# XiaoshuiHuang/GMF

Measured on AMD Instinct MI355X. Metric: correspondences/sec (whole node), higher is better.
Workload: dtype f32 (split-fp16 MFMA operands, fp32 accumulate; the cross products of the attention's two contractions, S = K Q'^T and O = P V, on block-scaled e4m3 operands wherever the device-side score guard allows)

## Files before the change

### gmf_amd/csrc/encoder_h2.hip

```cpp
#include <algorithm>
#include <cstdlib>
#include "enc_common.hpp"
#include "enc_ff.hpp"
#include "launchers.hpp"

namespace gmf {

#ifndef GMF_H2_RING
#define GMF_H2_RING 2
#endif
constexpr int kRing = GMF_H2_RING;

template <int MODE>
GMF_DEVINL void front_h2_body(float* lds, const int bx, const int pair, const int zsel_in, const float* __restrict__ in,
                              const float* __restrict__ wst, const float* __restrict__ vecs, float* __restrict__ f_out,
                              float* __restrict__ q_out, float* __restrict__ k_out, float* __restrict__ v_out, int N, int tiles,
                              const PairTab* __restrict__ ptab = nullptr, unsigned* __restrict__ v_scale = nullptr,
                              const PvGuard guard = {}) {
  const int lane = threadIdx.x & 63, h = lane >> 5, i = lane & 31;
  const int wave = __builtin_amdgcn_readfirstlane(threadIdx.x >> 6);
  const size_t row0 = pair_row0(ptab, pair, N);
  N = pair_rows(ptab, pair, N);
  const int tiles_p = ptab ? (N + 31) >> 5 : tiles;
  if (bx * kWavesPerWG >= tiles_p) return;
// ... 845 lines not shown
#pragma unroll
      for (int r = 0; r < 16; ++r) y[mb][r] = (x1[16 * mb + r] + b[r]) * 256.0f;
    }
  }
  __syncthreads();
  ff_chunks<NP>(nx, y, lds, ff_wst, lvec_f + 2 * C, lvec_f + 2 * C + FFH, wave, lane, h, 0, FFH / 32);
#pragma unroll
  for (int mb = 0; mb < 4; ++mb) {
    float t[16];
#pragma unroll
    for (int r = 0; r < 16; ++r) t[r] = y[mb][r] * kH2Inv;
    if (active) store_block_p32(x2_out + toff, mb, t, lane);
  }
}

template <int NP, bool QSKIP = false, bool KVF = false>
__global__ void __launch_bounds__(256, 2)
k_linear_h2(const float* __restrict__ f_in, const float* __restrict__ front_wst, const float* __restrict__ front_vec,
            const float* __restrict__ ctx_img, const float* __restrict__ attn_wst, const float* __restrict__ attn_vec,
            const float* __restrict__ ff_wst, const float* __restrict__ ff_vec, float* __restrict__ q_out,
            float* __restrict__ k_out, float* __restrict__ v_out, float* __restrict__ x2_out, int N, int tiles, int T,
            int ttiles, const PairTab* __restrict__ ptab, unsigned* __restrict__ v_scale, const PvGuard guard,
            const float* __restrict__ kvf_wst, const float* __restrict__ kvf_bias) {
  __shared__ __attribute__((aligned(16))) float lds[kLinLdsFloats];
  tail_priority(blockIdx.y * gridDim.x + blockIdx.x, gridDim.x * gridDim.y);
  linear_h2_body<0, NP, QSKIP, KVF>(lds, f_in, front_wst, front_vec, ctx_img, attn_wst, attn_vec, ff_wst, ff_vec, q_out, k_out, v_out, x2_out, N,
                                    tiles, T, ttiles, ptab, v_scale, guard, kvf_wst, kvf_bias);
}

template <bool KVF>
__global__ void __launch_bounds__(256, 2)
k_linear_roles(const float* __restrict__ f_in, const float* __restrict__ front_wst, const float* __restrict__ front_vec,
               const float* __restrict__ ctx_img, const float* __restrict__ attn_wst, const float* __restrict__ attn_vec,
               const float* __restrict__ ff_wst, const float* __restrict__ ff_vec, float* __restrict__ q_out,
               float* __restrict__ k_out, float* __restrict__ v_out, float* __restrict__ x2_out, int N, int tiles, int T,
               int ttiles, unsigned* __restrict__ v_scale, const PvGuard guard, const PairTab* __restrict__ ptab,
               const float* __restrict__ kvf_wst, const float* __restrict__ kvf_bias) {
  __shared__ __attribute__((aligned(16))) float lds[kLinLdsFloats];
  if (blockIdx.z == 0)
    linear_h2_body<1, 3, false, KVF>(lds, f_in, front_wst, front_vec, ctx_img, attn_wst, attn_vec, ff_wst, ff_vec, q_out, k_out, v_out, x2_out, N,
                                     tiles, T, ttiles, ptab, v_scale, guard, kvf_wst, kvf_bias);
  else
    linear_h2_body<2>(lds, f_in, front_wst, front_vec, ctx_img, attn_wst, attn_vec, ff_wst, ff_vec, q_out, k_out, v_out, x2_out, N,
                      tiles, T, ttiles, ptab);
}

__global__ void __launch_bounds__(256)
k_ff_reduce(const float* __restrict__ part, const float* __restrict__ x1, const float* __restrict__ vecs,
            float* __restrict__ x2_out, int tiles, int hs) {
  const int lane = threadIdx.x & 63, h = lane >> 5;
  const int tile = blockIdx.x * kWavesPerWG + (threadIdx.x >> 6);
  if (tile >= tiles) return;
  const int mb = blockIdx.z;
// ... 24 lines not shown
hipError_t launch_front_h2(int mode, bool split, const float* in, const float* wst, const float* vecs, float* f, float* q, float* k,
                           float* v, int B, int N, int tiles, hipStream_t s, const PairTab* ptab, unsigned* v_scale, PvGuard guard) {
  dim3 g = tgrid(tiles, B);
  if (split) g.z = 3;
  if (mode == 3) { g.z = 1; hipLaunchKernelGGL(k_front_h2<3>, g, dim3(256), 0, s, in, wst, vecs, f, q, k, v, N, tiles, ptab, v_scale, guard); }
  else if (mode == 1) hipLaunchKernelGGL(k_front_h2<1>, g, dim3(256), 0, s, in, wst, vecs, f, q, k, v, N, tiles, ptab, v_scale, guard);
  else if (mode == 2) hipLaunchKernelGGL(k_front_h2<2>, g, dim3(256), 0, s, in, wst, vecs, f, q, k, v, N, tiles, ptab, v_scale, guard);
  else hipLaunchKernelGGL(k_front_h2<0>, g, dim3(256), 0, s, in, wst, vecs, f, q, k, v, N, tiles, ptab, v_scale, guard);
  return hipGetLastError();
}

hipError_t launch_linear_h2(bool roles, const float* f, const float* front_wst, const float* front_vec, const float* ctx_img,
                            const float* attn_wst, const float* attn_vec, const float* ff_wst, const float* ff_vec, float* q,
                            float* k, float* v, float* x2, int B, int N, int tiles, int T, int ttiles, hipStream_t s,
                            bool one_product, const PairTab* ptab, unsigned* v_scale, PvGuard guard, const float* kvf_wst,
                            const float* kvf_bias) {
  const float* const none = nullptr;
  if (roles && kvf_wst)
    hipLaunchKernelGGL(k_linear_roles<true>, tgrid(tiles, B, 2), dim3(256), 0, s, f, front_wst, front_vec, ctx_img, attn_wst, attn_vec,
                       ff_wst, ff_vec, q, k, v, x2, N, tiles, T, ttiles, v_scale, guard, ptab, kvf_wst, kvf_bias);
  else if (roles)
    hipLaunchKernelGGL(k_linear_roles<false>, tgrid(tiles, B, 2), dim3(256), 0, s, f, front_wst, front_vec, ctx_img, attn_wst, attn_vec,
                       ff_wst, ff_vec, q, k, v, x2, N, tiles, T, ttiles, v_scale, guard, ptab, none, none);
  else if (kvf_wst && !q)
    hipLaunchKernelGGL((k_linear_h2<3, true, true>), tgrid(tiles, B), dim3(256), 0, s, f, front_wst, front_vec, ctx_img, attn_wst, attn_vec, ff_wst,
                       ff_vec, q, k, v, x2, N, tiles, T, ttiles, ptab, v_scale, guard, kvf_wst, kvf_bias);
  else if (kvf_wst)
    hipLaunchKernelGGL((k_linear_h2<3, false, true>), tgrid(tiles, B), dim3(256), 0, s, f, front_wst, front_vec, ctx_img, attn_wst, attn_vec, ff_wst,
                       ff_vec, q, k, v, x2, N, tiles, T, ttiles, ptab, v_scale, guard, kvf_wst, kvf_bias);
  else if (one_product)
    hipLaunchKernelGGL(k_linear_h2<1>, tgrid(tiles, B), dim3(256), 0, s, f, front_wst, front_vec, ctx_img, attn_wst, attn_vec, ff_wst,
                       ff_vec, q, k, v, x2, N, tiles, T, ttiles, ptab, v_scale, guard, none, none);
  else if (!q)
    hipLaunchKernelGGL((k_linear_h2<3, true>), tgrid(tiles, B), dim3(256), 0, s, f, front_wst, front_vec, ctx_img, attn_wst, attn_vec, ff_wst,
                       ff_vec, q, k, v, x2, N, tiles, T, ttiles, ptab, v_scale, guard, none, none);
  else
    hipLaunchKernelGGL(k_linear_h2<3>, tgrid(tiles, B), dim3(256), 0, s, f, front_wst, front_vec, ctx_img, attn_wst, attn_vec, ff_wst,
                       ff_vec, q, k, v, x2, N, tiles, T, ttiles, ptab, v_scale, guard, none, none);
  return hipGetLastError();
}

hipError_t launch_ctx_prep_h2(bool pe, const float* ctx, const float* wst, const float* vecs, float* out, int B, int T,
                              int ttiles, int sets, int wst_stride, int vec_stride, hipStream_t s, bool rowmajor) {
  if (pe) hipLaunchKernelGGL(k_ctx_prep_h2<true>, tgrid(ttiles, B, sets), dim3(256), 0, s, ctx, wst, vecs, out, T, ttiles, wst_stride, vec_stride);
  else if (rowmajor) hipLaunchKernelGGL((k_ctx_prep_h2<false, true>), tgrid(ttiles, B, sets), dim3(256), 0, s, ctx, wst, vecs, out, T, ttiles, wst_stride, vec_stride);
  else hipLaunchKernelGGL(k_ctx_prep_h2<false>, tgrid(ttiles, B, sets), dim3(256), 0, s, ctx, wst, vecs, out, T, ttiles, wst_stride, vec_stride);
  return hipGetLastError();
}

hipError_t launch_fusion_attn_h2(bool pe, const float* x, const float* ctx_img, const float* wst, const float* vecs,
                                 float* x1, int B, int N, int tiles, int T, int ttiles, hipStream_t s, bool rowmajor) {
  if (pe) hipLaunchKernelGGL(k_fusion_attn_h2<true>, tgrid(tiles, B), dim3(256), 0, s, x, ctx_img, wst, vecs, x1, N, tiles, T, ttiles);
  else if (rowmajor) hipLaunchKernelGGL((k_fusion_attn_h2<false, true>), tgrid(tiles, B), dim3(256), 0, s, x, ctx_img, wst, vecs, x1, N, tiles, T, ttiles);
// ... 72 lines not shown
```

### gmf_amd/csrc/encoder_kernels.hip

```cpp
#include <algorithm>
#include <type_traits>
#include "enc_common.hpp"
#include "enc_ff.hpp"

namespace gmf {

template <int MODE>
__global__ void __launch_bounds__(256, 2)
k_front(const float* __restrict__ in, const float* __restrict__ wst, const float* __restrict__ vecs,
        float* __restrict__ f_out, float* __restrict__ q_out, float* __restrict__ k_out,
        float* __restrict__ v_out, int N, int tiles) {
  __shared__ __attribute__((aligned(16))) float lds[2 * kStageFloats];
  const int lane = threadIdx.x & 63, wave = threadIdx.x >> 6, h = lane >> 5, i = lane & 31;
  const int pair = blockIdx.y;
  const int tile_raw = blockIdx.x * kWavesPerWG + wave;
  const bool active = tile_raw < tiles;
  const int tile = active ? tile_raw : tiles - 1;
  const size_t toff = ((size_t)pair * tiles + tile) * (32 * C);

  constexpr bool FIRST = (MODE == 1);
  StageStream ss;
  if (MODE == 2) ss.init(lds, lds + kStageFloats, wave, kWavesPerWG, lane, wst + 4 * kStageFloats, 12);
  else ss.init(lds, lds + kStageFloats, wave, kWavesPerWG, lane, wst, 16);
  ss.prime();
// ... 1064 lines not shown
  ss.prime();
  const FusTile ft{fus + toff};
  if (next_wst) scattn_epilogue_h2<true>(o, active, ss, lvec, ft, out + toff, lane, h, lvec + 2 * C, stat_next, pair,
                                         tile_raw * 32 + (lane & 31) < N);
  else scattn_epilogue_h2<false>(o, active, ss, lvec, ft, out + toff, lane, h);
}

GMF_DEVINL bool attn_pv_on(const unsigned* __restrict__ v_scale, const PvGuard& guard, int bid, int n_items, int n_full, int ksplits,
                           int wgs_per_pair, const PairTab* __restrict__ ptab = nullptr) {
  if (!guard.stat) return v_scale != nullptr;
  const AttnItem it = attn_item(bid, n_items, n_full, ksplits);
  const int slot = it.valid ? it.item / wgs_per_pair : 0;
  return pv_planes_on(v_scale, guard, ptab ? ptab[slot].ord : slot);
}

template <int NPROD, int CFMT, bool PVF8 = false, bool FOLD = false>
__global__ void __launch_bounds__(256, 2)
k_scattn_h2p(const float* __restrict__ q_img, const float* __restrict__ k_img, const float* __restrict__ v_img,
             const float* __restrict__ fus, const float* __restrict__ wst, const float* __restrict__ vecs,
             float* out, int N, int tiles, int wgs_per_pair, const float* __restrict__ c_dense,
             int n_items, int n_full, int ksplits, float* __restrict__ part_o, float* __restrict__ part_ml,
             const float* __restrict__ next_wst, const float* __restrict__ next_bias, const PairTab* __restrict__ ptab,
             const unsigned* __restrict__ v_scale, const float* qf_img, const float* __restrict__ qw_wst,
             const float* __restrict__ qw_bias, const PvGuard guard, const float* __restrict__ kvf_vec) {
  __shared__ __attribute__((aligned(16))) float lds[4 * kStageFloats];
  tail_priority(blockIdx.x, gridDim.x);
  if (!PVF8 || attn_pv_on(v_scale, guard, blockIdx.x, n_items, n_full, ksplits, wgs_per_pair, ptab))
    scattn_h2p_body<NPROD, CFMT, 4, PVF8, FOLD>(lds, blockIdx.x, q_img, k_img, v_img, fus, wst, vecs, out, N, tiles, wgs_per_pair, c_dense, n_items,
                                                n_full, ksplits, part_o, part_ml, next_wst, next_bias, ptab, v_scale, qf_img, qw_wst, qw_bias,
                                                guard.stat_next, kvf_vec);
  else
    scattn_h2p_body<NPROD, CFMT, 4, false, FOLD>(lds, blockIdx.x, q_img, k_img, v_img, fus, wst, vecs, out, N, tiles, wgs_per_pair, c_dense, n_items,
                                                 n_full, ksplits, part_o, part_ml, next_wst, next_bias, ptab, nullptr, qf_img, qw_wst, qw_bias,
                                                 guard.stat_next, kvf_vec);
}

__global__ void __launch_bounds__(256, 2)
k_scattn_fast(const float* __restrict__ q_img, const float* __restrict__ k_img, const float* __restrict__ v_img,
              const float* __restrict__ fus, const float* __restrict__ wst, const float* __restrict__ vecs,
              float* __restrict__ out, int N, int tiles, int wgs_per_pair, const float* __restrict__ c_half, int n_items,
              const float* __restrict__ next_wst, const float* __restrict__ next_bias) {
  constexpr int WAVES = 4;
  constexpr int kHiFloats = kStageFloats / 2;
  constexpr int kCFloats = 512;
  __shared__ __attribute__((aligned(16))) float lds[6 * kHiFloats + WAVES * 3 * kCFloats];
  float* const ldsK = lds;
  float* const ldsV = lds + 3 * kHiFloats;
  const int lane = threadIdx.x & 63, h = lane >> 5;
  const int wave = __builtin_amdgcn_readfirstlane(threadIdx.x >> 6);
// ... 908 lines not shown
                       tiles, ksplits, cc->next_wst_h2, cc->next_bias, (const float*)ff_part, ff_hs, x1, ff_vecs + 2 * C + 2 * FFH,
                       cc->guard.stat_next, N, cc->ptab);
  else
    hipLaunchKernelGGL(k_scattn_merge, dim3(8 * per_xcd), dim3(256), 0, s, cc->part_o, cc->part_ml, x1, cc->tail_wst_h2, tail_vecs, out,
                       tiles, wpp, W, 0, ksplits, cc->next_wst_h2, cc->next_bias, (const float*)ff_part, ff_hs, x1,
                       ff_vecs + 2 * C + 2 * FFH, cc->guard.stat_next, N, cc->ptab);
  return hipGetLastError();
}

hipError_t launch_scattn_h2p(const float* q, const float* k, const float* v, const float* fus, const float* vecs, float* out, int B,
                             int N, int tiles, hipStream_t s, const CompatCache& cc, int n_full, int ksplits) {
  const int wpp = (tiles + 3) / 4, W = wpp * B;
  const int per_xcd = (W >> 3) + ((W & 7) ? 1 : 0);
  const int max_tail = std::max(0, per_xcd - n_full);
  const dim3 grid(8 * (std::min(n_full, per_xcd) + max_tail * ksplits));
  if (cc.half && max_tail == 0)
    hipLaunchKernelGGL(k_scattn_fast, dim3(8 * per_xcd), dim3(256), 0, s, q, k, v, fus, cc.tail_wst_h2, vecs, out, N, tiles, wpp, cc.dense, W,
                       cc.next_wst_h2, cc.next_bias);
  else if (cc.half)
    hipLaunchKernelGGL((k_scattn_h2p<1, 1>), grid, dim3(256), 0, s, q, k, v, fus, cc.tail_wst_h2, vecs, out, N, tiles, wpp, cc.dense, W,
                       n_full, ksplits, cc.part_o, cc.part_ml, cc.next_wst_h2, cc.next_bias, cc.ptab, (const unsigned*)nullptr, (const float*)nullptr, (const float*)nullptr, (const float*)nullptr, PvGuard{}, (const float*)nullptr);
  else if (cc.fmt == 2 && cc.v_scale)
    hipLaunchKernelGGL((k_scattn_h2p<3, 2, true>), grid, dim3(256), 0, s, q, k, v, fus, cc.tail_wst_h2, vecs, out, N, tiles, wpp, cc.dense,
                       W, n_full, ksplits, cc.part_o, cc.part_ml, cc.next_wst_h2, cc.next_bias, cc.ptab, cc.v_scale, cc.qf_img, cc.qw_wst, cc.qw_bias, cc.guard, (const float*)nullptr);
  else if (cc.fmt == 2)
    hipLaunchKernelGGL((k_scattn_h2p<3, 2>), grid, dim3(256), 0, s, q, k, v, fus, cc.tail_wst_h2, vecs, out, N, tiles, wpp, cc.dense,
                       W, n_full, ksplits, cc.part_o, cc.part_ml, cc.next_wst_h2, cc.next_bias, cc.ptab, (const unsigned*)nullptr, cc.qf_img, cc.qw_wst, cc.qw_bias, PvGuard{}, (const float*)nullptr);
  else if (cc.kvf_vec && cc.v_scale)
    hipLaunchKernelGGL((k_scattn_h2p<3, 0, true, true>), grid, dim3(256), 0, s, q, k, v, fus, cc.tail_wst_h2, vecs, out, N, tiles, wpp, cc.dense,
                       W, n_full, ksplits, cc.part_o, cc.part_ml, cc.next_wst_h2, cc.next_bias, cc.ptab, cc.v_scale, cc.qf_img, cc.qw_wst, cc.qw_bias, cc.guard, cc.kvf_vec);
  else if (cc.kvf_vec)
    hipLaunchKernelGGL((k_scattn_h2p<3, 0, false, true>), grid, dim3(256), 0, s, q, k, v, fus, cc.tail_wst_h2, vecs, out, N, tiles, wpp, cc.dense,
                       W, n_full, ksplits, cc.part_o, cc.part_ml, cc.next_wst_h2, cc.next_bias, cc.ptab, (const unsigned*)nullptr, cc.qf_img, cc.qw_wst, cc.qw_bias, PvGuard{}, cc.kvf_vec);
  else if (cc.v_scale)
    hipLaunchKernelGGL((k_scattn_h2p<3, 0, true>), grid, dim3(256), 0, s, q, k, v, fus, cc.tail_wst_h2, vecs, out, N, tiles, wpp, cc.dense,
                       W, n_full, ksplits, cc.part_o, cc.part_ml, cc.next_wst_h2, cc.next_bias, cc.ptab, cc.v_scale, cc.qf_img, cc.qw_wst, cc.qw_bias, cc.guard, (const float*)nullptr);
  else
    hipLaunchKernelGGL((k_scattn_h2p<3, 0>), grid, dim3(256), 0, s, q, k, v, fus, cc.tail_wst_h2, vecs, out, N, tiles, wpp, cc.dense,
                       W, n_full, ksplits, cc.part_o, cc.part_ml, cc.next_wst_h2, cc.next_bias, cc.ptab, (const unsigned*)nullptr, cc.qf_img, cc.qw_wst, cc.qw_bias, PvGuard{}, (const float*)nullptr);
  if (max_tail > 0)
    hipLaunchKernelGGL(k_scattn_merge, dim3(8 * max_tail), dim3(256), 0, s, cc.part_o, cc.part_ml, fus, cc.tail_wst_h2, vecs, out,
                       tiles, wpp, W, n_full, ksplits, cc.next_wst_h2, cc.next_bias, (const float*)nullptr, 0,
                       (const float*)nullptr, (const float*)nullptr, cc.guard.stat_next, N, cc.ptab);
  return hipGetLastError();
}

hipError_t launch_scattn_h2(const float* q, const float* k, const float* v, const float* pts8, const float* fus, const float* wst,
                            const float* vecs, float* out, int B, int N, int tiles, float sigma_d, hipStream_t s, const float* c_dense) {
  const float inv = 1.0f / (sigma_d * sigma_d);
  const int wpp = (tiles + 3) / 4;
  if (c_dense) hipLaunchKernelGGL(k_scattn_h2<true>, dim3(wpp * B), dim3(256), 0, s, q, k, v, pts8, fus, wst, vecs, out, N, tiles, inv, wpp, c_dense);
  else hipLaunchKernelGGL(k_scattn_h2<false>, dim3(wpp * B), dim3(256), 0, s, q, k, v, pts8, fus, wst, vecs, out, N, tiles, inv, wpp, c_dense);
  return hipGetLastError();
}
// ... 79 lines not shown
```

### gmf_amd/csrc/gmf_api.cpp

```cpp
#include "../../include/gmf_hip.h"

#include <hip/hip_runtime.h>

#include <cmath>
#include <cstdint>
#include <cstdio>
#include <algorithm>
#include <cstring>
#include <new>
#include <string>
#include <utility>
#include <vector>

#include "api_common.hpp"
#include "launchers_pose.hpp"
#include "launchers_solvers.hpp"
#include "launchers_spectral.hpp"
#include "launchers_pointcloud.hpp"
#include "launchers_sparse.hpp"
#include "launchers_dgr_input.hpp"
#include "launchers_correspondence.hpp"
#include "launchers_posegraph.hpp"
#include "launchers_clique.hpp"
#include "launchers_tsdf.hpp"
// ... 273 lines not shown
  if (std::strcmp(name, "kv_fold") == 0) {
    GMF_REQUIRE(value == 0 || value == 1, GMF_ERR_BAD_ARG, "set_tuning: kv_fold must be 0 or 1");
    t.kv_fold = value != 0;
    return GMF_OK;
  }
  if (std::strcmp(name, "pv_fp8") == 0) {
    GMF_REQUIRE(value >= 0 && value <= 2, GMF_ERR_BAD_ARG, "set_tuning: pv_fp8 must be 0 (three f16 products), 1 (guarded, default) or 2 (always)");
    t.pv_fp8 = value;
    return GMF_OK;
  }
  if (std::strcmp(name, "compat_format") == 0) {
    GMF_REQUIRE(value == 0 || value == 2, GMF_ERR_BAD_ARG, "set_tuning: compat_format must be 0 (fp32) or 2 (16-bit fixed point of c)");
    t.compat_format = value;
    return GMF_OK;
  }
  if (std::strcmp(name, "precision") == 0) {
    GMF_REQUIRE(value >= 0 && value <= 2, GMF_ERR_BAD_ARG, "set_tuning: precision must be 0 (parity), 1 or 2 (throughput numerics)");
    t.precision = value;
    return GMF_OK;
  }
  if (std::strcmp(name, "spectral_col_splits") == 0) {
    GMF_REQUIRE(value >= 0 && value <= gmf::kSmMaxSplits, GMF_ERR_BAD_ARG, "set_tuning: spectral_col_splits out of range (0..32)");
    t.spectral_col_splits = value;
    return GMF_OK;
  }
  if (std::strcmp(name, "clique_local_rows") == 0) {
    GMF_REQUIRE(value >= 0 && value <= gmf::kPmcLocal, GMF_ERR_BAD_ARG, "set_tuning: clique_local_rows out of range (0..384)");
    t.clique_local_rows = value;
    return GMF_OK;
  }
  return fail(h, GMF_ERR_BAD_ARG, std::string("gmf: set_tuning: unknown knob ") + name);
}

int gmf_get_tuning(gmf_handle* h, const char* name, int* value) {
  GMF_REQUIRE(h && name && value, GMF_ERR_BAD_ARG, "get_tuning: null pointer");
  std::lock_guard<std::mutex> lock(h->mu);
  const gmf::Tuning& t = h->tune;
  const struct { const char* name; int v; } tab[] = {
      {"scattn_variant", t.scattn_variant}, {"front_output_split", t.front_split ? 1 : 0}, {"ff_hidden_splits", t.ff_split},
      {"attn_key_splits", t.key_splits}, {"attn_tail_split", t.tail_split ? 1 : 0}, {"small_grid_roles", t.small_roles ? 1 : 0},
      {"fused_linear", t.fused_linear ? 1 : 0}, {"compat_cache", t.use_cache ? 1 : 0}, {"conv_lds_patch", t.conv_patch}, {"conv_small_grid", t.conv_small ? 1 : 0}, {"small_prologue_roles", t.small_prologue ? 1 : 0}, {"small_fattn_tile", t.small_fattn_tile ? 1 : 0},
      {"nms_binned", t.nms_binned}, {"topk_select", t.topk_select ? 1 : 0}, {"wide_attn_tile", t.wide_attn_tile ? 1 : 0},
      {"small_merge_tile", t.small_merge_tile ? 1 : 0}, {"mid_grid_roles", t.mid_grid_roles}, {"pv_fp8", t.pv_fp8}, {"q_in_attention", t.q_in_attention ? 1 : 0},
      {"kv_fold", t.kv_fold ? 1 : 0}, {"compat_format", t.compat_format}, {"precision", t.precision}, {"spectral_col_splits", t.spectral_col_splits},
      {"clique_local_rows", t.clique_local_rows}};
  for (const auto& e : tab) {
    if (std::strcmp(name, e.name) == 0) { *value = e.v; return GMF_OK; }
  }
  return fail(h, GMF_ERR_BAD_ARG, std::string("gmf: get_tuning: unknown knob ") + name);
}

int gmf_profile_enable(gmf_handle* h, int on) {
  GMF_REQUIRE(h, GMF_ERR_BAD_ARG, "profile_enable: null handle");
  h->profile = (on != 0);
  h->prof_used = 0;
  return GMF_OK;
}

int gmf_profile_read(gmf_handle* h, double* scattn_ms_total, int* scattn_launches) {
// ... 189 lines not shown
  bool fused() const { return form >= kFusedStages; }
  bool f1_h2 = false;
  bool prologue = false;
  bool cache = false;
  bool pipelined = false;
  int fmt = 0;
  bool half = false;
  bool one_product = false;
  bool front_split = false;
  int max_splits = 0;
  int attn_nf = 0, attn_ks = 1;
  int ff_hs = 1, f1_ff_hs = 1;
  bool roles = false;
  bool q_in_attn = false;
  bool kv_fold = false;
  bool v_fp8 = false;
  bool guard = false;
  bool clear_stats = false;
  size_t act = 0, tok = 0, cache_floats = 0;
};

static EncoderPlan plan_encoder(const gmf::Tuning& t, const gmf_encoder_weights* w, int B, int N, int T, int L, int min_tiles, int cus,
                                bool dense = false) {
  EncoderPlan p;
  const int tiles = tiles_of(N), tt = tiles_of(T);
  const int W = ((tiles + 3) / 4) * B;
  const bool ragged = min_tiles > 0;
  p.act = (size_t)B * tiles * kTileFloats;
  p.tok = (size_t)B * tt * kTileFloats;
  const bool h2 = !dense && t.scattn_variant >= 9 && w->front_wst_h2 && w->ctx_wst_h2 && w->attn_wst_h2 && w->ff_wst_h2 && w->tail_wst_h2;
  const bool fusable = h2 && t.fused_linear && t.scattn_variant == 18;
  const bool half = t.precision >= 1 && fusable && W >= 256 && !ragged;
  const int fmt = half ? 1 : t.scattn_variant == 18 ? t.compat_format : 0;
  const size_t cache_floats = (size_t)B * tiles * tiles * (fmt ? 512 : 1024);
  p.cache = h2 && L > 1 && t.use_cache && cache_floats * 4 <= ((size_t)96 << 30);
  const bool fused = fusable && p.cache;
  if (p.cache) { p.cache_floats = cache_floats; p.fmt = fmt; p.half = half; }
  p.one_product = p.half && t.precision == 2;
  p.pipelined = p.cache && t.scattn_variant == 18;
  p.front_split = t.front_split && W < 128;
  p.max_splits = (p.cache && tiles >= 8) ? (W < 384 ? 8 : 4) : 0;
  plan_attn_split(t, cus, W, ragged ? min_tiles : tiles, p.max_splits, ragged, &p.attn_nf, &p.attn_ks);
  p.ff_hs = plan_ff_split(t, W, p.max_splits);
  p.f1_ff_hs = tt <= tiles ? plan_ff_split(t, ((tt + 3) / 4) * B, p.max_splits) : 1;
  if (!h2) p.form = EncoderPlan::kFp32;
  else if (!fused) p.form = EncoderPlan::kStages;
  else if (W < 256 && t.small_roles && p.attn_nf == 0 && p.attn_ks > 1 && p.ff_hs > 1 && p.max_splits == 8) p.form = EncoderPlan::kSmall3;
  else p.form = (W >= 256 || ragged) ? EncoderPlan::kLinear : EncoderPlan::kFusedStages;
  p.roles = p.form == EncoderPlan::kLinear && t.mid_grid_roles > 0 && W < t.mid_grid_roles;
  p.q_in_attn = p.form == EncoderPlan::kLinear && t.q_in_attention && !p.half && !p.roles;
  p.kv_fold = t.kv_fold && p.form == EncoderPlan::kLinear && p.pipelined && !p.half && p.fmt == 0 && w->kv_fold != nullptr;
  p.v_fp8 = fused && !p.half && (t.pv_fp8 == 2 || (t.pv_fp8 == 1 && w->pv_guard));
  p.clear_stats = fused && t.pv_fp8 == 1 && w->pv_guard;
  p.guard = p.clear_stats && !p.half;
  p.f1_h2 = h2 && w->f1_ctx_wst_h2 && w->f1_attn_wst_h2 && w->f1_ff_wst_h2;
  p.prologue = t.small_prologue && fused && p.f1_h2 && p.fmt == 0 && W < 256;
  return p;
}

static int prof_begin(gmf_handle* h, hipStream_t st, hipEvent_t* ev0, hipEvent_t* ev1) {
  *ev0 = *ev1 = nullptr;
  if (!h->profile) return GMF_OK;
  if (h->prof_used == h->prof_events.size()) {
    hipEvent_t a, b;
    GMF_HIP(hipEventCreate(&a));
    GMF_HIP(hipEventCreate(&b));
    h->prof_events.emplace_back(a, b);
  }
  *ev0 = h->prof_events[h->prof_used].first;
  *ev1 = h->prof_events[h->prof_used].second;
  ++h->prof_used;
// ... 80 lines not shown
  if (ragged) {
    long long n_sum = 0;
    if (int rc = check_ragged_sizes(h, n_points, B)) return rc;
    if (int rc = ring_take(h, tab, &ring)) return rc;
    gmf::plan_pair_table(n_points, B, -1.0, 0, pairs.host(ring.host), &N, &n_sum, nullptr);
    min_tiles = tiles_of(*std::min_element(n_points, n_points + B));
  }
  const int L = w->num_layers;
  const int tiles = tiles_of(N), tt = tiles_of(T);
  const EncoderPlan p = plan_encoder(h->tune, w, B, N, T, L, min_tiles, cu_count());
  GMF_REQUIRE(p.fused() || !ragged, GMF_ERR_UNSUPPORTED_SHAPE,
              "encoder_forward_ragged: ragged batches run on the default path only (split-fp16 weight images, at least two layers, the "
              "compat cache, \"fused_linear\" = 1, \"scattn_variant\" = 18)");
  const size_t act = p.act, tok = p.tok;
  char* dtab;
  float *featA, *featB, *f, *q, *k, *v, *x1, *x2, *pts8, *pimg, *qimg, *f1ctx, *x1t, *imgfeat, *ctxall, *c_dense, *ff_part, *part_o,
      *part_ml;
  unsigned *v_scale, *fstat;
  if (int rc = arena_carve(h, {arena_buf(dtab, tab.bytes()), arena_buf(featA, act), arena_buf(featB, act), arena_buf(f, act),
                               arena_buf(q, act), arena_buf(k, act), arena_buf(v, act), arena_buf(x1, act), arena_buf(x2, act),
                               arena_buf(pts8, (size_t)B * tiles * 32 * 8), arena_buf(pimg, tok), arena_buf(qimg, tok),
                               arena_buf(f1ctx, tok), arena_buf(x1t, tok), arena_buf(imgfeat, tok),
                               arena_buf(ctxall, (size_t)(L > 0 ? L : 1) * tok),
                               arena_buf(v_scale, (size_t)B * tiles * 128),
                               arena_buf(fstat, (size_t)(L + 1) * B * gmf::kPvStatStride),
                               arena_buf(c_dense, p.cache_floats),
                               arena_buf(ff_part, p.max_splits == 8 ? 8 * act : 0),
                               arena_buf(part_o, p.max_splits * act),
                               arena_buf(part_ml, (size_t)p.max_splits * B * tiles * 64)}))
    return rc;
  if (int rc = ragged ? ring_upload(h, ring, dtab, st) : GMF_OK) return rc;
  const gmf::PairTab* const ptab = ragged ? pairs.dev(dtab) : nullptr;
  gmf::CompatCache cc{c_dense, nullptr, part_o, part_ml};
  cc.half = p.half;
  cc.fmt = p.fmt;
  cc.ptab = ptab;
  cc.v_scale = p.v_fp8 ? v_scale : nullptr;
  unsigned* const zero_words = p.clear_stats ? fstat : nullptr;
  const int n_zero = p.clear_stats ? (L + 1) * B * gmf::kPvStatStride : 0;
  if (p.prologue) {
    GMF_HIP(gmf::launch_pro_ctx_pts(p_tokens, w->f1_ctx_wst_h2, w->f1_ctx_vec, f1ctx, B, T, tt, src_keypts, tgt_keypts, pts8, N, st, ptab,
                                    zero_words, n_zero));
    GMF_HIP(gmf::launch_pro_fattn_compat(q_tokens, f1ctx, w->f1_attn_wst_h2, w->f1_attn_vec, x1t, B, T, tt, pts8, c_dense, N, tiles,
                                         w->sigma_d, st, ptab));
    gmf::PvGuard g0;
    if (p.guard) g0.stat_next = fstat;
    GMF_HIP(gmf::launch_pro_ff_front(x1t, w->f1_ff_wst_h2, w->f1_ff_vec, imgfeat, B, tt, part_o, p.f1_ff_hs, corr_pos, w->front_wst_h2,
                                     w->front_vec, f, q, k, v, N, tiles, st, ptab, g0));
    if (p.f1_ff_hs > 1) GMF_HIP(gmf::launch_ff_reduce_h2(part_o, x1t, w->f1_ff_vec, imgfeat, B, tt, p.f1_ff_hs, st));
    GMF_HIP(gmf::launch_ctx_prep_h2(true, imgfeat, w->ctx_wst_h2, w->ctx_vec, ctxall, B, T, tt, L, w->ctx_wst_stride, w->ctx_vec_stride, st));
// ... 44 lines not shown
      cc.next_bias = last ? nullptr : w->front_vec + (size_t)(l + 1) * w->front_vec_stride;
      if (p.form == EncoderPlan::kLinear) {
        cc.qf_img = p.q_in_attn ? f : nullptr;
        cc.qw_wst = p.q_in_attn ? fw + 4 * kTileFloats : nullptr;
        cc.qw_bias = p.q_in_attn ? fv + kC : nullptr;
        const float* kvf = p.kv_fold ? w->kv_fold + (size_t)l * GMF_KV_FOLD_STRIDE : nullptr;
        const float* kvf_vecs = kvf ? kvf + 9 * kTileFloats : nullptr;
        if (kvf) {
          cc.qf_img = f;
          cc.qw_wst = p.q_in_attn ? kvf : nullptr;
          cc.qw_bias = p.q_in_attn ? kvf_vecs : nullptr;
          cc.tail_wst_h2 = kvf + 4 * kTileFloats;
          cc.kvf_vec = kvf_vecs + kC;
          tail_vecs = kvf_vecs + 3 * kC;
        }
        GMF_HIP(gmf::launch_linear_h2(p.roles, f, fw, fv, ctx_l, aw, av, ffw, ffv, p.q_in_attn ? nullptr : q, k, v, x2, B, N, tiles, T, tt,
                                      st, p.one_product, ptab, cc.v_scale, cc.guard, kvf, kvf_vecs));
      } else if (p.form == EncoderPlan::kSmall3) {
        GMF_HIP(gmf::launch_small_front_fattn(f, fw, fv, ctx_l, aw, av, q, k, v, x1, B, N, tiles, T, tt, st, cc.v_scale, cc.guard,
                                              h->tune.small_fattn_tile, ptab));
        hipEvent_t e0 = nullptr, e1 = nullptr;
        if (int rc = prof_begin(h, st, &e0, &e1)) return rc;
        GMF_HIP(gmf::launch_small_attn_ff_merge(q, k, v, x1, ffw, ffv, ff_part, p.ff_hs, w->tail_vec + (size_t)l * w->tail_vec_stride,
                                                last ? cur : f, B, N, tiles, p.attn_ks, st, &cc, h->tune.small_merge_tile));
        if (e1) GMF_HIP(hipEventRecord(e1, st));
        continue;
      } else {
        GMF_HIP(gmf::launch_front_h2(2, p.front_split, f, fw, fv, f, q, k, v, B, N, tiles, st, nullptr, cc.v_scale, cc.guard));
        GMF_HIP(gmf::launch_fusion_attn_h2(true, f, ctx_l, aw, av, x1, B, N, tiles, T, tt, st));
        GMF_HIP(gmf::launch_fusion_ff_h2(x1, ffw, ffv, x2, B, tiles, st, part_o, p.ff_hs));
      }
      if (int rc = run_scattn(h, w, p, l, q, k, v, pts8, x2, last ? cur : f, B, N, st, nullptr, cc, tail_vecs)) return rc;
// ... 1298 lines not shown
```

### gmf_amd/csrc/launchers.hpp

```cpp
#pragma once
#include <hip/hip_runtime.h>

#include "pair_plan.hpp"

namespace gmf {


constexpr int kPvStatStride = 32;
struct PvGuard {
  const unsigned* stat = nullptr;
  const float* thr2 = nullptr;
  unsigned* stat_next = nullptr;
};

struct CompatCache {
  const float* dense;
  const float* tail_wst_h2;
  float* part_o;
  float* part_ml;
  const float* next_wst_h2 = nullptr;
  const float* next_bias = nullptr;
  bool half = false;
  const PairTab* ptab = nullptr;
  int fmt = 0;
  unsigned* v_scale = nullptr;
  const float* qf_img = nullptr;
  const float* qw_wst = nullptr;
  const float* qw_bias = nullptr;
  PvGuard guard;
  const float* kvf_vec = nullptr;
};

struct Tuning {
  int scattn_variant = 18;
  bool use_cache = true;
  int key_splits = 0;
  bool tail_split = false;
  int ff_split = 0;
  bool front_split = true;
  bool wide_attn_tile = true;
  bool small_merge_tile = true;
  bool small_fattn_tile = true;
  bool small_roles = true;
  bool fused_linear = true;
  int conv_patch = 1;
  bool small_prologue = true;
  bool conv_small = true;
  int nms_binned = 1;
  bool topk_select = true;
  int mid_grid_roles = 512;
  bool kv_fold = true;
  bool q_in_attention = true;
  int pv_fp8 = 1;
  int compat_format = 0;
  int precision = 0;
  int spectral_col_splits = 0;
  int clique_local_rows = 384;
};

hipError_t launch_compat_build(const float* pts8, float* c_dense, int B, int N, int tiles, float sigma_d, int fmt, hipStream_t s,
                               const PairTab* ptab = nullptr);
hipError_t launch_front(int mode, const float* in, const float* wst, const float* vecs, float* f, float* q, float* k,
                        float* v, int B, int N, int tiles, hipStream_t s);
hipError_t launch_scattn_fp32(const float* q, const float* k, const float* v, const float* pts8, const float* fus,
                              const float* wst, const float* vecs, float* out, int B, int N, int tiles, float sigma_d,
                              hipStream_t s);
hipError_t launch_scattn_h2(const float* q, const float* k, const float* v, const float* pts8, const float* fus, const float* wst,
                            const float* vecs, float* out, int B, int N, int tiles, float sigma_d, hipStream_t s, const float* c_dense);
hipError_t launch_scattn_h2p(const float* q, const float* k, const float* v, const float* fus, const float* vecs, float* out, int B,
// ... 16 lines not shown
hipError_t launch_ctx_prep_w_h2(bool pe, const float* ctx, const float* wst_h2, const float* vecs, float* out, int B, int T,
                                int ttiles, hipStream_t s, bool rowmajor = false);
hipError_t launch_fusion_attn_w_h2(bool pe, const float* x, const float* ctx_img, const float* wst_h2, const float* vecs,
                                   float* x1, int B, int N, int tiles, int T, int ttiles, hipStream_t s, bool tile_form = true);
hipError_t launch_fusion_ff_w_h2(const float* x1, const float* wst_h2, const float* vecs, float* x2, int B, int tiles, hipStream_t s,
                                 float* part = nullptr, int hs = 1, float* out_rm = nullptr, long o_sb = 0, long o_sr = 0,
                                 long o_sk = 0, int n_rows = 0, int* status = nullptr);
int plan_ff_split_w(int base_wgs);
hipError_t launch_front_h2(int mode, bool split, const float* in, const float* wst, const float* vecs, float* f, float* q, float* k,
                           float* v, int B, int N, int tiles, hipStream_t s, const PairTab* ptab = nullptr, unsigned* v_scale = nullptr,
                           PvGuard guard = {});
hipError_t launch_linear_h2(bool roles, const float* f, const float* front_wst, const float* front_vec, const float* ctx_img,
                            const float* attn_wst, const float* attn_vec, const float* ff_wst, const float* ff_vec, float* q,
                            float* k, float* v, float* x2, int B, int N, int tiles, int T, int ttiles, hipStream_t s, bool one_product = false,
                            const PairTab* ptab = nullptr, unsigned* v_scale = nullptr, PvGuard guard = {}, const float* kvf_wst = nullptr,
                            const float* kvf_bias = nullptr);
hipError_t launch_small_front_fattn(const float* f, const float* front_wst, const float* front_vec, const float* ctx_img,
                                    const float* attn_wst, const float* attn_vec, float* q, float* k, float* v, float* x1, int B,
                                    int N, int tiles, int T, int ttiles, hipStream_t s, unsigned* v_scale = nullptr, PvGuard guard = {},
                                    bool tile_role = true, const PairTab* ptab = nullptr);
hipError_t launch_small_attn_ff_merge(const float* q, const float* k, const float* v, const float* x1, const float* ff_wst,
                                      const float* ff_vecs, float* ff_part, int ff_hs, const float* tail_vecs, float* out, int B,
                                      int N, int tiles, int ksplits, hipStream_t s, const CompatCache* cc, bool tile_merge = true);
hipError_t launch_ctx_prep_h2(bool pe, const float* ctx, const float* wst, const float* vecs, float* out, int B, int T,
                              int ttiles, int sets, int wst_stride, int vec_stride, hipStream_t s, bool rowmajor = false);
hipError_t launch_fusion_attn_h2(bool pe, const float* x, const float* ctx_img, const float* wst, const float* vecs,
                                 float* x1, int B, int N, int tiles, int T, int ttiles, hipStream_t s, bool rowmajor = false);
hipError_t launch_pro_ctx_pts(const float* p_tokens, const float* wst, const float* vecs, float* f1ctx, int B, int T, int ttiles,
                              const float* src, const float* tgt, float* pts8, int N, hipStream_t s, const PairTab* ptab,
                              unsigned* zero_words, int n_zero);
hipError_t launch_pro_fattn_compat(const float* q_tokens, const float* f1ctx, const float* wst, const float* vecs, float* x1t, int B,
// ... 88 lines not shown
```

Baseline: 10.05 million.

## Store compat cache in 16-bit format with lazily built fp32 fallback for guard trips

When the PV fp8 path is on, the linear-form encoder now uses the half-size 16-bit compatibility cache format instead of fp32, and lets kv_fold combine with it. Because the fp8 guard's fallback path needs the fp32 cache, a second fp32 buffer is allocated and filled lazily by an extra grid z-slice of the linear kernel, only for pairs whose guard first trips at the current layer. The aim is to halve cache bandwidth in attention, at the cost of extra memory, an extra block role in the linear launch, and a rebuild of the fallback cache on the layer where the guard trips.

```diff
diff --git a/gmf_amd/csrc/encoder_h2.hip b/gmf_amd/csrc/encoder_h2.hip
--- a/gmf_amd/csrc/encoder_h2.hip
+++ b/gmf_amd/csrc/encoder_h2.hip
@@ -883,6 +883,17 @@
   }
 }
 
+GMF_DEVINL void compat_tripped_role(float* tr, const LazyCompat& lz, int N, int tiles, const PairTab* __restrict__ ptab) {
+  const int pair = blockIdx.y, B = gridDim.y;
+  auto trips = [&](int l) { return !(__uint_as_float(lz.fstat[((size_t)l * B + pair) * kPvStatStride]) <= lz.thr2[l]); };
+  if (!trips(lz.layer)) return;
+  for (int l = 0; l < lz.layer; ++l)
+    if (trips(l)) return;
+  const int gy = (tiles + 4 * kJPerWave - 1) / (4 * kJPerWave);
+  for (int w = blockIdx.x; w < tiles * gy; w += gridDim.x)
+    compat_build_body<0>(tr, w % tiles, w / tiles, pair, lz.pts8, lz.c_dense, N, tiles, lz.inv_sig2, ptab);
+}
+
 template <int NP, bool QSKIP = false, bool KVF = false>
 __global__ void __launch_bounds__(256, 2)
 k_linear_h2(const float* __restrict__ f_in, const float* __restrict__ front_wst, const float* __restrict__ front_vec,
@@ -890,8 +901,10 @@
             const float* __restrict__ ff_wst, const float* __restrict__ ff_vec, float* __restrict__ q_out,
             float* __restrict__ k_out, float* __restrict__ v_out, float* __restrict__ x2_out, int N, int tiles, int T,
             int ttiles, const PairTab* __restrict__ ptab, unsigned* __restrict__ v_scale, const PvGuard guard,
-            const float* __restrict__ kvf_wst, const float* __restrict__ kvf_bias) {
+            const float* __restrict__ kvf_wst, const float* __restrict__ kvf_bias, const LazyCompat lazy) {
   __shared__ __attribute__((aligned(16))) float lds[kLinLdsFloats];
+  static_assert(kLinLdsFloats >= kCompatLdsFloats, "the compat role's transposes fit the kernel's LDS");
+  if (blockIdx.z == 1) return compat_tripped_role(lds, lazy, N, tiles, ptab);
   tail_priority(blockIdx.y * gridDim.x + blockIdx.x, gridDim.x * gridDim.y);
   linear_h2_body<0, NP, QSKIP, KVF>(lds, f_in, front_wst, front_vec, ctx_img, attn_wst, attn_vec, ff_wst, ff_vec, q_out, k_out, v_out, x2_out, N,
                                     tiles, T, ttiles, ptab, v_scale, guard, kvf_wst, kvf_bias);
@@ -904,8 +917,9 @@
                const float* __restrict__ ff_wst, const float* __restrict__ ff_vec, float* __restrict__ q_out,
                float* __restrict__ k_out, float* __restrict__ v_out, float* __restrict__ x2_out, int N, int tiles, int T,
                int ttiles, unsigned* __restrict__ v_scale, const PvGuard guard, const PairTab* __restrict__ ptab,
-               const float* __restrict__ kvf_wst, const float* __restrict__ kvf_bias) {
+               const float* __restrict__ kvf_wst, const float* __restrict__ kvf_bias, const LazyCompat lazy) {
   __shared__ __attribute__((aligned(16))) float lds[kLinLdsFloats];
+  if (blockIdx.z == 2) return compat_tripped_role(lds, lazy, N, tiles, ptab);
   if (blockIdx.z == 0)
     linear_h2_body<1, 3, false, KVF>(lds, f_in, front_wst, front_vec, ctx_img, attn_wst, attn_vec, ff_wst, ff_vec, q_out, k_out, v_out, x2_out, N,
                                      tiles, T, ttiles, ptab, v_scale, guard, kvf_wst, kvf_bias);
@@ -960,29 +974,30 @@
                             const float* attn_wst, const float* attn_vec, const float* ff_wst, const float* ff_vec, float* q,
                             float* k, float* v, float* x2, int B, int N, int tiles, int T, int ttiles, hipStream_t s,
                             bool one_product, const PairTab* ptab, unsigned* v_scale, PvGuard guard, const float* kvf_wst,
-                            const float* kvf_bias) {
+                            const float* kvf_bias, LazyCompat lazy) {
   const float* const none = nullptr;
+  const int lz = lazy.c_dense ? 1 : 0;
   if (roles && kvf_wst)
-    hipLaunchKernelGGL(k_linear_roles<true>, tgrid(tiles, B, 2), dim3(256), 0, s, f, front_wst, front_vec, ctx_img, attn_wst, attn_vec,
-                       ff_wst, ff_vec, q, k, v, x2, N, tiles, T, ttiles, v_scale, guard, ptab, kvf_wst, kvf_bias);
+    hipLaunchKernelGGL(k_linear_roles<true>, tgrid(tiles, B, 2 + lz), dim3(256), 0, s, f, front_wst, front_vec, ctx_img, attn_wst, attn_vec,
+                       ff_wst, ff_vec, q, k, v, x2, N, tiles, T, ttiles, v_scale, guard, ptab, kvf_wst, kvf_bias, lazy);
   else if (roles)
-    hipLaunchKernelGGL(k_linear_roles<false>, tgrid(tiles, B, 2), dim3(256), 0, s, f, front_wst, front_vec, ctx_img, attn_wst, attn_vec,
-                       ff_wst, ff_vec, q, k, v, x2, N, tiles, T, ttiles, v_scale, guard, ptab, none, none);
+    hipLaunchKernelGGL(k_linear_roles<false>, tgrid(tiles, B, 2 + lz), dim3(256), 0, s, f, front_wst, front_vec, ctx_img, attn_wst, attn_vec,
+                       ff_wst, ff_vec, q, k, v, x2, N, tiles, T, ttiles, v_scale, guard, ptab, none, none, lazy);
   else if (kvf_wst && !q)
-    hipLaunchKernelGGL((k_linear_h2<3, true, true>), tgrid(tiles, B), dim3(256), 0, s, f, front_wst, front_vec, ctx_img, attn_wst, attn_vec, ff_wst,
-                       ff_vec, q, k, v, x2, N, tiles, T, ttiles, ptab, v_scale, guard, kvf_wst, kvf_bias);
+    hipLaunchKernelGGL((k_linear_h2<3, true, true>), tgrid(tiles, B, 1 + lz), dim3(256), 0, s, f, front_wst, front_vec, ctx_img, attn_wst, attn_vec, ff_wst,
+                       ff_vec, q, k, v, x2, N, tiles, T, ttiles, ptab, v_scale, guard, kvf_wst, kvf_bias, lazy);
   else if (kvf_wst)
-    hipLaunchKernelGGL((k_linear_h2<3, false, true>), tgrid(tiles, B), dim3(256), 0, s, f, front_wst, front_vec, ctx_img, attn_wst, attn_vec, ff_wst,
-                       ff_vec, q, k, v, x2, N, tiles, T, ttiles, ptab, v_scale, guard, kvf_wst, kvf_bias);
+    hipLaunchKernelGGL((k_linear_h2<3, false, true>), tgrid(tiles, B, 1 + lz), dim3(256), 0, s, f, front_wst, front_vec, ctx_img, attn_wst, attn_vec, ff_wst,
+                       ff_vec, q, k, v, x2, N, tiles, T, ttiles, ptab, v_scale, guard, kvf_wst, kvf_bias, lazy);
   else if (one_product)
-    hipLaunchKernelGGL(k_linear_h2<1>, tgrid(tiles, B), dim3(256), 0, s, f, front_wst, front_vec, ctx_img, attn_wst, attn_vec, ff_wst,
-                       ff_vec, q, k, v, x2, N, tiles, T, ttiles, ptab, v_scale, guard, none, none);
+    hipLaunchKernelGGL(k_linear_h2<1>, tgrid(tiles, B, 1 + lz), dim3(256), 0, s, f, front_wst, front_vec, ctx_img, attn_wst, attn_vec, ff_wst,
+                       ff_vec, q, k, v, x2, N, tiles, T, ttiles, ptab, v_scale, guard, none, none, lazy);
   else if (!q)
-    hipLaunchKernelGGL((k_linear_h2<3, true>), tgrid(tiles, B), dim3(256), 0, s, f, front_wst, front_vec, ctx_img, attn_wst, attn_vec, ff_wst,
-                       ff_vec, q, k, v, x2, N, tiles, T, ttiles, ptab, v_scale, guard, none, none);
+    hipLaunchKernelGGL((k_linear_h2<3, true>), tgrid(tiles, B, 1 + lz), dim3(256), 0, s, f, front_wst, front_vec, ctx_img, attn_wst, attn_vec, ff_wst,
+                       ff_vec, q, k, v, x2, N, tiles, T, ttiles, ptab, v_scale, guard, none, none, lazy);
   else
-    hipLaunchKernelGGL(k_linear_h2<3>, tgrid(tiles, B), dim3(256), 0, s, f, front_wst, front_vec, ctx_img, attn_wst, attn_vec, ff_wst,
-                       ff_vec, q, k, v, x2, N, tiles, T, ttiles, ptab, v_scale, guard, none, none);
+    hipLaunchKernelGGL(k_linear_h2<3>, tgrid(tiles, B, 1 + lz), dim3(256), 0, s, f, front_wst, front_vec, ctx_img, attn_wst, attn_vec, ff_wst,
+                       ff_vec, q, k, v, x2, N, tiles, T, ttiles, ptab, v_scale, guard, none, none, lazy);
   return hipGetLastError();
 }
 
diff --git a/gmf_amd/csrc/encoder_kernels.hip b/gmf_amd/csrc/encoder_kernels.hip
--- a/gmf_amd/csrc/encoder_kernels.hip
+++ b/gmf_amd/csrc/encoder_kernels.hip
@@ -1102,7 +1102,7 @@
   return pv_planes_on(v_scale, guard, ptab ? ptab[slot].ord : slot);
 }
 
-template <int NPROD, int CFMT, bool PVF8 = false, bool FOLD = false>
+template <int NPROD, int CFMT, bool PVF8 = false, bool FOLD = false, int CFB = CFMT>
 __global__ void __launch_bounds__(256, 2)
 k_scattn_h2p(const float* __restrict__ q_img, const float* __restrict__ k_img, const float* __restrict__ v_img,
              const float* __restrict__ fus, const float* __restrict__ wst, const float* __restrict__ vecs,
@@ -1110,7 +1110,9 @@
              int n_items, int n_full, int ksplits, float* __restrict__ part_o, float* __restrict__ part_ml,
              const float* __restrict__ next_wst, const float* __restrict__ next_bias, const PairTab* __restrict__ ptab,
              const unsigned* __restrict__ v_scale, const float* qf_img, const float* __restrict__ qw_wst,
-             const float* __restrict__ qw_bias, const PvGuard guard, const float* __restrict__ kvf_vec) {
+             const float* __restrict__ qw_bias, const PvGuard guard, const float* __restrict__ kvf_vec,
+             const float* __restrict__ c_dense_fb) {
+  static_assert(CFB == CFMT || PVF8, "a second cache format belongs to the guarded fp8 form");
   __shared__ __attribute__((aligned(16))) float lds[4 * kStageFloats];
   tail_priority(blockIdx.x, gridDim.x);
   if (!PVF8 || attn_pv_on(v_scale, guard, blockIdx.x, n_items, n_full, ksplits, wgs_per_pair, ptab))
@@ -1118,9 +1120,10 @@
                                                 n_full, ksplits, part_o, part_ml, next_wst, next_bias, ptab, v_scale, qf_img, qw_wst, qw_bias,
                                                 guard.stat_next, kvf_vec);
   else
-    scattn_h2p_body<NPROD, CFMT, 4, false, FOLD>(lds, blockIdx.x, q_img, k_img, v_img, fus, wst, vecs, out, N, tiles, wgs_per_pair, c_dense, n_items,
-                                                 n_full, ksplits, part_o, part_ml, next_wst, next_bias, ptab, nullptr, qf_img, qw_wst, qw_bias,
-                                                 guard.stat_next, kvf_vec);
+    scattn_h2p_body<NPROD, CFB, 4, false, FOLD>(lds, blockIdx.x, q_img, k_img, v_img, fus, wst, vecs, out, N, tiles, wgs_per_pair,
+                                                CFB == CFMT ? c_dense : c_dense_fb, n_items,
+                                                n_full, ksplits, part_o, part_ml, next_wst, next_bias, ptab, nullptr, qf_img, qw_wst, qw_bias,
+                                                guard.stat_next, kvf_vec);
 }
 
 __global__ void __launch_bounds__(256, 2)
@@ -2059,30 +2062,27 @@
   const int per_xcd = (W >> 3) + ((W & 7) ? 1 : 0);
   const int max_tail = std::max(0, per_xcd - n_full);
   const dim3 grid(8 * (std::min(n_full, per_xcd) + max_tail * ksplits));
+  auto go = [&](auto kern, bool pvf8) {
+    hipLaunchKernelGGL(kern, grid, dim3(256), 0, s, q, k, v, fus, cc.tail_wst_h2, vecs, out, N, tiles, wpp, cc.dense, W, n_full, ksplits,
+                       cc.part_o, cc.part_ml, cc.next_wst_h2, cc.next_bias, cc.ptab, pvf8 ? (const unsigned*)cc.v_scale : nullptr, cc.qf_img,
+                       cc.qw_wst, cc.qw_bias, pvf8 ? cc.guard : PvGuard{}, cc.kvf_vec, cc.dense_fb);
+  };
+  const bool pvf8 = cc.v_scale != nullptr, fold = cc.kvf_vec != nullptr;
   if (cc.half && max_tail == 0)
     hipLaunchKernelGGL(k_scattn_fast, dim3(8 * per_xcd), dim3(256), 0, s, q, k, v, fus, cc.tail_wst_h2, vecs, out, N, tiles, wpp, cc.dense, W,
                        cc.next_wst_h2, cc.next_bias);
   else if (cc.half)
-    hipLaunchKernelGGL((k_scattn_h2p<1, 1>), grid, dim3(256), 0, s, q, k, v, fus, cc.tail_wst_h2, vecs, out, N, tiles, wpp, cc.dense, W,
-                       n_full, ksplits, cc.part_o, cc.part_ml, cc.next_wst_h2, cc.next_bias, cc.ptab, (const unsigned*)nullptr, (const float*)nullptr, (const float*)nullptr, (const float*)nullptr, PvGuard{}, (const float*)nullptr);
-  else if (cc.fmt == 2 && cc.v_scale)
-    hipLaunchKernelGGL((k_scattn_h2p<3, 2, true>), grid, dim3(256), 0, s, q, k, v, fus, cc.tail_wst_h2, vecs, out, N, tiles, wpp, cc.dense,
-                       W, n_full, ksplits, cc.part_o, cc.part_ml, cc.next_wst_h2, cc.next_bias, cc.ptab, cc.v_scale, cc.qf_img, cc.qw_wst, cc.qw_bias, cc.guard, (const float*)nullptr);
+    go(k_scattn_h2p<1, 1>, false);
+  else if (cc.fmt == 2 && cc.dense_fb && pvf8)
+    fold ? go(k_scattn_h2p<3, 2, true, true, 0>, true) : go(k_scattn_h2p<3, 2, true, false, 0>, true);
+  else if (cc.fmt == 2 && pvf8)
+    fold ? go(k_scattn_h2p<3, 2, true, true>, true) : go(k_scattn_h2p<3, 2, true>, true);
   else if (cc.fmt == 2)
-    hipLaunchKernelGGL((k_scattn_h2p<3, 2>), grid, dim3(256), 0, s, q, k, v, fus, cc.tail_wst_h2, vecs, out, N, tiles, wpp, cc.dense,
-                       W, n_full, ksplits, cc.part_o, cc.part_ml, cc.next_wst_h2, cc.next_bias, cc.ptab, (const unsigned*)nullptr, cc.qf_img, cc.qw_wst, cc.qw_bias, PvGuard{}, (const float*)nullptr);
-  else if (cc.kvf_vec && cc.v_scale)
-    hipLaunchKernelGGL((k_scattn_h2p<3, 0, true, true>), grid, dim3(256), 0, s, q, k, v, fus, cc.tail_wst_h2, vecs, out, N, tiles, wpp, cc.dense,
-                       W, n_full, ksplits, cc.part_o, cc.part_ml, cc.next_wst_h2, cc.next_bias, cc.ptab, cc.v_scale, cc.qf_img, cc.qw_wst, cc.qw_bias, cc.guard, cc.kvf_vec);
-  else if (cc.kvf_vec)
-    hipLaunchKernelGGL((k_scattn_h2p<3, 0, false, true>), grid, dim3(256), 0, s, q, k, v, fus, cc.tail_wst_h2, vecs, out, N, tiles, wpp, cc.dense,
-                       W, n_full, ksplits, cc.part_o, cc.part_ml, cc.next_wst_h2, cc.next_bias, cc.ptab, (const unsigned*)nullptr, cc.qf_img, cc.qw_wst, cc.qw_bias, PvGuard{}, cc.kvf_vec);
-  else if (cc.v_scale)
-    hipLaunchKernelGGL((k_scattn_h2p<3, 0, true>), grid, dim3(256), 0, s, q, k, v, fus, cc.tail_wst_h2, vecs, out, N, tiles, wpp, cc.dense,
-                       W, n_full, ksplits, cc.part_o, cc.part_ml, cc.next_wst_h2, cc.next_bias, cc.ptab, cc.v_scale, cc.qf_img, cc.qw_wst, cc.qw_bias, cc.guard, (const float*)nullptr);
+    fold ? go(k_scattn_h2p<3, 2, false, true>, false) : go(k_scattn_h2p<3, 2>, false);
+  else if (pvf8)
+    fold ? go(k_scattn_h2p<3, 0, true, true>, true) : go(k_scattn_h2p<3, 0, true>, true);
   else
-    hipLaunchKernelGGL((k_scattn_h2p<3, 0>), grid, dim3(256), 0, s, q, k, v, fus, cc.tail_wst_h2, vecs, out, N, tiles, wpp, cc.dense,
-                       W, n_full, ksplits, cc.part_o, cc.part_ml, cc.next_wst_h2, cc.next_bias, cc.ptab, (const unsigned*)nullptr, cc.qf_img, cc.qw_wst, cc.qw_bias, PvGuard{}, (const float*)nullptr);
+    fold ? go(k_scattn_h2p<3, 0, false, true>, false) : go(k_scattn_h2p<3, 0>, false);
   if (max_tail > 0)
     hipLaunchKernelGGL(k_scattn_merge, dim3(8 * max_tail), dim3(256), 0, s, cc.part_o, cc.part_ml, fus, cc.tail_wst_h2, vecs, out,
                        tiles, wpp, W, n_full, ksplits, cc.next_wst_h2, cc.next_bias, (const float*)nullptr, 0,
diff --git a/gmf_amd/csrc/gmf_api.cpp b/gmf_amd/csrc/gmf_api.cpp
--- a/gmf_amd/csrc/gmf_api.cpp
+++ b/gmf_amd/csrc/gmf_api.cpp
@@ -311,6 +311,11 @@
     t.compat_format = value;
     return GMF_OK;
   }
+  if (std::strcmp(name, "compat_16") == 0) {
+    GMF_REQUIRE(value >= 0 && value <= 2, GMF_ERR_BAD_ARG, "set_tuning: compat_16 must be 0, 1 or 2");
+    t.compat_16 = value;
+    return GMF_OK;
+  }
   if (std::strcmp(name, "precision") == 0) {
     GMF_REQUIRE(value >= 0 && value <= 2, GMF_ERR_BAD_ARG, "set_tuning: precision must be 0 (parity), 1 or 2 (throughput numerics)");
     t.precision = value;
@@ -339,7 +344,7 @@
       {"fused_linear", t.fused_linear ? 1 : 0}, {"compat_cache", t.use_cache ? 1 : 0}, {"conv_lds_patch", t.conv_patch}, {"conv_small_grid", t.conv_small ? 1 : 0}, {"small_prologue_roles", t.small_prologue ? 1 : 0}, {"small_fattn_tile", t.small_fattn_tile ? 1 : 0},
       {"nms_binned", t.nms_binned}, {"topk_select", t.topk_select ? 1 : 0}, {"wide_attn_tile", t.wide_attn_tile ? 1 : 0},
       {"small_merge_tile", t.small_merge_tile ? 1 : 0}, {"mid_grid_roles", t.mid_grid_roles}, {"pv_fp8", t.pv_fp8}, {"q_in_attention", t.q_in_attention ? 1 : 0},
-      {"kv_fold", t.kv_fold ? 1 : 0}, {"compat_format", t.compat_format}, {"precision", t.precision}, {"spectral_col_splits", t.spectral_col_splits},
+      {"kv_fold", t.kv_fold ? 1 : 0}, {"compat_format", t.compat_format}, {"compat_16", t.compat_16}, {"precision", t.precision}, {"spectral_col_splits", t.spectral_col_splits},
       {"clique_local_rows", t.clique_local_rows}};
   for (const auto& e : tab) {
     if (std::strcmp(name, e.name) == 0) { *value = e.v; return GMF_OK; }
@@ -559,10 +564,12 @@
   bool roles = false;
   bool q_in_attn = false;
   bool kv_fold = false;
+  bool c16_guard = false;
   bool v_fp8 = false;
   bool guard = false;
   bool clear_stats = false;
   size_t act = 0, tok = 0, cache_floats = 0;
+  size_t cache_fb_floats = 0;
 };
 
 static EncoderPlan plan_encoder(const gmf::Tuning& t, const gmf_encoder_weights* w, int B, int N, int T, int L, int min_tiles, int cus,
@@ -578,7 +585,8 @@
   const bool half = t.precision >= 1 && fusable && W >= 256 && !ragged;
   const int fmt = half ? 1 : t.scattn_variant == 18 ? t.compat_format : 0;
   const size_t cache_floats = (size_t)B * tiles * tiles * (fmt ? 512 : 1024);
-  p.cache = h2 && L > 1 && t.use_cache && cache_floats * 4 <= ((size_t)96 << 30);
+  const size_t cache_cap = (size_t)96 << 30;
+  p.cache = h2 && L > 1 && t.use_cache && cache_floats * 4 <= cache_cap;
   const bool fused = fusable && p.cache;
   if (p.cache) { p.cache_floats = cache_floats; p.fmt = fmt; p.half = half; }
   p.one_product = p.half && t.precision == 2;
@@ -594,12 +602,23 @@
   else p.form = (W >= 256 || ragged) ? EncoderPlan::kLinear : EncoderPlan::kFusedStages;
   p.roles = p.form == EncoderPlan::kLinear && t.mid_grid_roles > 0 && W < t.mid_grid_roles;
   p.q_in_attn = p.form == EncoderPlan::kLinear && t.q_in_attention && !p.half && !p.roles;
-  p.kv_fold = t.kv_fold && p.form == EncoderPlan::kLinear && p.pipelined && !p.half && p.fmt == 0 && w->kv_fold != nullptr;
+  p.f1_h2 = h2 && w->f1_ctx_wst_h2 && w->f1_attn_wst_h2 && w->f1_ff_wst_h2;
+  const bool pro_grid = t.small_prologue && fused && p.f1_h2 && W < 256;
+  if ((t.compat_16 == 2 || (t.compat_16 == 1 && W >= 256)) && p.form == EncoderPlan::kLinear && p.pipelined && !p.half && p.fmt == 0 &&
+      (t.pv_fp8 == 2 || (t.pv_fp8 == 1 && w->pv_guard))) {
+    const size_t fb = t.pv_fp8 == 1 ? cache_floats : 0;
+    if ((cache_floats / 2 + fb) * 4 <= cache_cap) {
+      p.fmt = 2;
+      p.cache_floats = cache_floats / 2;
+      p.cache_fb_floats = fb;
+      p.c16_guard = fb != 0;
+    }
+  }
+  p.kv_fold = t.kv_fold && p.form == EncoderPlan::kLinear && p.pipelined && !p.half && w->kv_fold != nullptr;
   p.v_fp8 = fused && !p.half && (t.pv_fp8 == 2 || (t.pv_fp8 == 1 && w->pv_guard));
   p.clear_stats = fused && t.pv_fp8 == 1 && w->pv_guard;
   p.guard = p.clear_stats && !p.half;
-  p.f1_h2 = h2 && w->f1_ctx_wst_h2 && w->f1_attn_wst_h2 && w->f1_ff_wst_h2;
-  p.prologue = t.small_prologue && fused && p.f1_h2 && p.fmt == 0 && W < 256;
+  p.prologue = pro_grid && p.fmt == 0;
   return p;
 }
 
@@ -710,8 +729,8 @@
               "compat cache, \"fused_linear\" = 1, \"scattn_variant\" = 18)");
   const size_t act = p.act, tok = p.tok;
   char* dtab;
-  float *featA, *featB, *f, *q, *k, *v, *x1, *x2, *pts8, *pimg, *qimg, *f1ctx, *x1t, *imgfeat, *ctxall, *c_dense, *ff_part, *part_o,
-      *part_ml;
+  float *featA, *featB, *f, *q, *k, *v, *x1, *x2, *pts8, *pimg, *qimg, *f1ctx, *x1t, *imgfeat, *ctxall, *c_dense, *c_dense_fb, *ff_part,
+      *part_o, *part_ml;
   unsigned *v_scale, *fstat;
   if (int rc = arena_carve(h, {arena_buf(dtab, tab.bytes()), arena_buf(featA, act), arena_buf(featB, act), arena_buf(f, act),
                                arena_buf(q, act), arena_buf(k, act), arena_buf(v, act), arena_buf(x1, act), arena_buf(x2, act),
@@ -721,6 +740,7 @@
                                arena_buf(v_scale, (size_t)B * tiles * 128),
                                arena_buf(fstat, (size_t)(L + 1) * B * gmf::kPvStatStride),
                                arena_buf(c_dense, p.cache_floats),
+                               arena_buf(c_dense_fb, p.cache_fb_floats),
                                arena_buf(ff_part, p.max_splits == 8 ? 8 * act : 0),
                                arena_buf(part_o, p.max_splits * act),
                                arena_buf(part_ml, (size_t)p.max_splits * B * tiles * 64)}))
@@ -730,6 +750,7 @@
   gmf::CompatCache cc{c_dense, nullptr, part_o, part_ml};
   cc.half = p.half;
   cc.fmt = p.fmt;
+  cc.dense_fb = p.c16_guard ? c_dense_fb : nullptr;
   cc.ptab = ptab;
   cc.v_scale = p.v_fp8 ? v_scale : nullptr;
   unsigned* const zero_words = p.clear_stats ? fstat : nullptr;
@@ -804,8 +825,10 @@
           cc.kvf_vec = kvf_vecs + kC;
           tail_vecs = kvf_vecs + 3 * kC;
         }
+        gmf::LazyCompat lazy;
+        if (p.c16_guard) lazy = gmf::LazyCompat{c_dense_fb, pts8, fstat, w->pv_guard, l, 1.0f / (w->sigma_d * w->sigma_d)};
         GMF_HIP(gmf::launch_linear_h2(p.roles, f, fw, fv, ctx_l, aw, av, ffw, ffv, p.q_in_attn ? nullptr : q, k, v, x2, B, N, tiles, T, tt,
-                                      st, p.one_product, ptab, cc.v_scale, cc.guard, kvf, kvf_vecs));
+                                      st, p.one_product, ptab, cc.v_scale, cc.guard, kvf, kvf_vecs, lazy));
       } else if (p.form == EncoderPlan::kSmall3) {
         GMF_HIP(gmf::launch_small_front_fattn(f, fw, fv, ctx_l, aw, av, q, k, v, x1, B, N, tiles, T, tt, st, cc.v_scale, cc.guard,
                                               h->tune.small_fattn_tile, ptab));
diff --git a/gmf_amd/csrc/launchers.hpp b/gmf_amd/csrc/launchers.hpp
--- a/gmf_amd/csrc/launchers.hpp
+++ b/gmf_amd/csrc/launchers.hpp
@@ -29,6 +29,16 @@
   const float* qw_bias = nullptr;
   PvGuard guard;
   const float* kvf_vec = nullptr;
+  const float* dense_fb = nullptr;
+};
+
+struct LazyCompat {
+  float* c_dense = nullptr;
+  const float* pts8 = nullptr;
+  const unsigned* fstat = nullptr;
+  const float* thr2 = nullptr;
+  int layer = 0;
+  float inv_sig2 = 0.f;
 };
 
 struct Tuning {
@@ -53,6 +63,7 @@
   bool q_in_attention = true;
   int pv_fp8 = 1;
   int compat_format = 0;
+  int compat_16 = 1;
   int precision = 0;
   int spectral_col_splits = 0;
   int clique_local_rows = 384;
@@ -99,7 +110,7 @@
                             const float* attn_wst, const float* attn_vec, const float* ff_wst, const float* ff_vec, float* q,
                             float* k, float* v, float* x2, int B, int N, int tiles, int T, int ttiles, hipStream_t s, bool one_product = false,
                             const PairTab* ptab = nullptr, unsigned* v_scale = nullptr, PvGuard guard = {}, const float* kvf_wst = nullptr,
-                            const float* kvf_bias = nullptr);
+                            const float* kvf_bias = nullptr, LazyCompat lazy = {});
 hipError_t launch_small_front_fattn(const float* f, const float* front_wst, const float* front_vec, const float* ctx_img,
                                     const float* attn_wst, const float* attn_vec, float* q, float* k, float* v, float* x1, int B,
                                     int N, int tiles, int T, int ttiles, hipStream_t s, unsigned* v_scale = nullptr, PvGuard guard = {},
```

New measurement: 10.96 million (median of 6 runs). 1.09x the previous value.
